# StefanSko/mcmc-db

Hardware: AMD Instinct MI355X
Metric: validated param-draws/sec (higher is better)
Workload: dtype f64; 1 GPU; single posteriordb-shaped model, 4x10000x100 synthetic draws per GPU (BASELINE config 1; AR(1) chains, ties and a shifted chain; SURVEY 8(d) C1); layout=pcn, statistics=mean,std,q5,q50,q95,split_rhat,ess_bulk,ess_tail

## Files before the change

### mcmc-db_amd/csrc/mcr_device.hpp

```cpp
#pragma once
#include <hip/hip_runtime.h>
#include <stdint.h>

namespace mcr {

using i64 = long long;
using u32 = unsigned int;
using u64 = unsigned long long;

constexpr int kWave = 64;

template <int CTRL>
__device__ __forceinline__ double dpp_f64(double v)
{
    const int lo = __builtin_amdgcn_mov_dpp(__double2loint(v), CTRL, 0xf, 0xf, true);
    const int hi = __builtin_amdgcn_mov_dpp(__double2hiint(v), CTRL, 0xf, 0xf, true);
    return __hiloint2double(hi, lo);
}
__device__ __forceinline__ double readlane_f64(double v, int lane)
{
    return __hiloint2double(__builtin_amdgcn_readlane(__double2hiint(v), lane),
                            __builtin_amdgcn_readlane(__double2loint(v), lane));
}
constexpr int kDppXor1 = 0xB1, kDppXor2 = 0x4E, kDppRor4 = 0x124, kDppRor8 = 0x128;

__device__ __forceinline__ double row_sum(double v)
{
    v += dpp_f64<kDppXor1>(v); v += dpp_f64<kDppXor2>(v); v += dpp_f64<kDppRor4>(v); v += dpp_f64<kDppRor8>(v);
    return v;
}
template <int CTRL>
__device__ __forceinline__ u32 dpp_u32(u32 v) { return (u32)__builtin_amdgcn_mov_dpp((int)v, CTRL, 0xf, 0xf, true); }
__device__ __forceinline__ u32 row_min_u32(u32 v)
{
    v = min(v, dpp_u32<kDppXor1>(v)); v = min(v, dpp_u32<kDppXor2>(v));
    v = min(v, dpp_u32<kDppRor4>(v)); v = min(v, dpp_u32<kDppRor8>(v));
    return v;
}
__device__ __forceinline__ u32 row_max_u32(u32 v)
{
    v = max(v, dpp_u32<kDppXor1>(v)); v = max(v, dpp_u32<kDppXor2>(v));
    v = max(v, dpp_u32<kDppRor4>(v)); v = max(v, dpp_u32<kDppRor8>(v));
    return v;
}
__device__ __forceinline__ double wave_sum(double v)
{
    v = row_sum(v);
    return (readlane_f64(v, 0) + readlane_f64(v, 16)) + (readlane_f64(v, 32) + readlane_f64(v, 48));
}
template <int CTRL, int ROW_MASK>
__device__ __forceinline__ double dpp_f64_or_zero(double v)
{
    const int lo = __builtin_amdgcn_update_dpp(0, __double2loint(v), CTRL, ROW_MASK, 0xf, false);
    const int hi = __builtin_amdgcn_update_dpp(0, __double2hiint(v), CTRL, ROW_MASK, 0xf, false);
    return __hiloint2double(hi, lo);
}
__device__ __forceinline__ double wave_excl_scan(double v, double& total)
{
    double incl = v;
    incl += dpp_f64_or_zero<0x111, 0xf>(incl);
    incl += dpp_f64_or_zero<0x112, 0xf>(incl);
    incl += dpp_f64_or_zero<0x114, 0xf>(incl);
    incl += dpp_f64_or_zero<0x118, 0xf>(incl);
    incl += dpp_f64_or_zero<0x142, 0xa>(incl);
    incl += dpp_f64_or_zero<0x143, 0xc>(incl);
    total = readlane_f64(incl, 63);
    return incl - v;
}

__device__ __forceinline__ int row_lane(int v, int j)
{
#define MCR_RL(J) case J: return __builtin_amdgcn_update_dpp(0, v, 0x150 + J, 0xf, 0xf, false);
    switch (j & 15) {
        MCR_RL(0) MCR_RL(1) MCR_RL(2) MCR_RL(3) MCR_RL(4) MCR_RL(5) MCR_RL(6) MCR_RL(7)
        MCR_RL(8) MCR_RL(9) MCR_RL(10) MCR_RL(11) MCR_RL(12) MCR_RL(13) MCR_RL(14)
        default: return __builtin_amdgcn_update_dpp(0, v, 0x15F, 0xf, 0xf, false);
    }
#undef MCR_RL
}

template <int CTRL, int ROW_MASK, int OLD>
__device__ __forceinline__ int dpp_i32_or(int v) { return __builtin_amdgcn_update_dpp(OLD, v, CTRL, ROW_MASK, 0xf, false); }

__device__ __forceinline__ u32 wave_excl_scan_u32(u32 v, u32& total)
{
    int incl = (int)v;
    incl += dpp_i32_or<0x111, 0xf, 0>(incl); incl += dpp_i32_or<0x112, 0xf, 0>(incl);
    incl += dpp_i32_or<0x114, 0xf, 0>(incl); incl += dpp_i32_or<0x118, 0xf, 0>(incl);
    incl += dpp_i32_or<0x142, 0xa, 0>(incl);
    incl += dpp_i32_or<0x143, 0xc, 0>(incl);
    total = (u32)__builtin_amdgcn_readlane(incl, 63);
    return (u32)incl - v;
}

__device__ __forceinline__ int wave_prefix_max(int v, int& excl)
{
    v = max(v, dpp_i32_or<0x111, 0xf, -1>(v)); v = max(v, dpp_i32_or<0x112, 0xf, -1>(v));
    v = max(v, dpp_i32_or<0x114, 0xf, -1>(v)); v = max(v, dpp_i32_or<0x118, 0xf, -1>(v));
    v = max(v, dpp_i32_or<0x142, 0xa, -1>(v)); v = max(v, dpp_i32_or<0x143, 0xc, -1>(v));
    excl = dpp_i32_or<0x138, 0xf, -1>(v);
    return v;
}
__device__ __forceinline__ int wave_suffix_min(int v, int& excl)
{
    constexpr int kMax = 0x7fffffff;
    v = min(v, dpp_i32_or<0x101, 0xf, kMax>(v)); v = min(v, dpp_i32_or<0x102, 0xf, kMax>(v));
    v = min(v, dpp_i32_or<0x104, 0xf, kMax>(v)); v = min(v, dpp_i32_or<0x108, 0xf, kMax>(v));
    const int r1 = __builtin_amdgcn_readlane(v, 16), r2 = __builtin_amdgcn_readlane(v, 32), r3 = __builtin_amdgcn_readlane(v, 48);
    const int row = (threadIdx.x & 63) >> 4;
    const int m23 = min(r2, r3), m123 = min(r1, m23);
    const int above = (row == 0) ? m123 : ((row == 1) ? m23 : ((row == 2) ? r3 : kMax));
    v = min(v, above);
    excl = dpp_i32_or<0x130, 0xf, kMax>(v);
    return v;
}

template <int NT>
__device__ __forceinline__ double block_sum(double v, double* red)
{
    v = wave_sum(v);
    __syncthreads();
    if ((threadIdx.x & 63) == 0) red[threadIdx.x >> 6] = v;
    __syncthreads();
    double r = 0.0;
#pragma unroll
    for (int w = 0; w < NT / kWave; ++w) r += red[w];
    return r;
}

template <int NT>
__device__ __forceinline__ void block_sum3(double& a, double& b, double& c, double* red)
{
    constexpr int NW = NT / kWave;
    a = wave_sum(a); b = wave_sum(b); c = wave_sum(c);
    __syncthreads();
    if ((threadIdx.x & 63) == 0) {
        const int w = threadIdx.x >> 6;
        red[w] = a; red[NW + w] = b; red[2 * NW + w] = c;
    }
    __syncthreads();
    double ra = 0.0, rb = 0.0, rc = 0.0;
#pragma unroll
    for (int w = 0; w < NW; ++w) { ra += red[w]; rb += red[NW + w]; rc += red[2 * NW + w]; }
    a = ra; b = rb; c = rc;
    __syncthreads();
}

__device__ __noinline__ double inv_cdf(double p)
{
#pragma clang fp contract(off)
    double q = p - 0.5, r, num, den, x;
    if (fabs(q) <= 0.425) {
        r = 0.180625 - q * q;
        num = (((((((2.5090809287301226727e+3 * r + 3.3430575583588128105e+4) * r +
                    6.7265770927008700853e+4) * r + 4.5921953931549871457e+4) * r +
                  1.3731693765509461125e+4) * r + 1.9715909503065514427e+3) * r +
                1.3314166789178437745e+2) * r + 3.3871328727963666080e+0) * q;
        den = (((((((5.2264952788528545610e+3 * r + 2.8729085735721942674e+4) * r +
                    3.9307895800092710610e+4) * r + 2.1213794301586595867e+4) * r +
                  5.3941960214247511077e+3) * r + 6.8718700749205790830e+2) * r +
                4.2313330701600911252e+1) * r + 1.0);
        return num / den;
    }
    r = (q <= 0.0) ? p : 1.0 - p;
    r = sqrt(-log(r));
    if (r <= 5.0) {
        r = r - 1.6;
        num = (((((((7.74545014278341407640e-4 * r + 2.27238449892691845833e-2) * r +
                    2.41780725177450611770e-1) * r + 1.27045825245236838258e+0) * r +
                  3.64784832476320460504e+0) * r + 5.76949722146069140550e+0) * r +
                4.63033784615654529590e+0) * r + 1.42343711074968357734e+0);
        den = (((((((1.05075007164441684324e-9 * r + 5.47593808499534494600e-4) * r +
                    1.51986665636164571966e-2) * r + 1.48103976427480074590e-1) * r +
                  6.89767334985100004550e-1) * r + 1.67638483018380384940e+0) * r +
                2.05319162663775882187e+0) * r + 1.0);
    } else {
        r = r - 5.0;
        num = (((((((2.01033439929228813265e-7 * r + 2.71155556874348757815e-5) * r +
                    1.24266094738807843860e-3) * r + 2.65321895265761230930e-2) * r +
                  2.96560571828504891230e-1) * r + 1.78482653991729133580e+0) * r +
                5.46378491116411436990e+0) * r + 6.65790464350110377720e+0);
        den = (((((((2.04426310338993978564e-15 * r + 1.42151175831644588870e-7) * r +
                    1.84631831751005468180e-5) * r + 7.86869131145613259100e-4) * r +
                  1.48753612908506148525e-2) * r + 1.36929880922735805310e-1) * r +
                5.99832206555887937690e-1) * r + 1.0);
    }
    x = num / den;
    return (q < 0.0) ? -x : x;
}

template <class FA, class FB>
__device__ __forceinline__ i64 merge_path(FA a, i64 na, FB b, i64 nb, i64 diag)
{
    i64 lo = diag > nb ? diag - nb : 0;
    i64 hi = diag < na ? diag : na;
    while (lo < hi) {
        i64 mid = (lo + hi) >> 1;
        const auto ak = a(mid), bk = b(diag - 1 - mid);
        if (!(bk < ak)) lo = mid + 1; else hi = mid;
    }
    return lo;
}

template <class FA, class FB>
__device__ __forceinline__ int merge_path32(FA a, int na, FB b, int nb, int diag)
{
    int lo = diag > nb ? diag - nb : 0;
    int hi = diag < na ? diag : na;
    while (lo < hi) {
        const int mid = (lo + hi) >> 1;
        const auto ak = a(mid), bk = b(diag - 1 - mid);
        const bool right = !(bk < ak);
        lo = right ? mid + 1 : lo;
        hi = right ? hi : mid;
    }
    return lo;
}

template <class FA, class FB>
__device__ __forceinline__ i64 merge_path_wave(FA a, i64 na, FB b, i64 nb, i64 diag)
{
    const int lane = threadIdx.x & 63;
    i64 lo = diag > nb ? diag - nb : 0;
    i64 hi = diag < na ? diag : na;
    while (lo < hi) {
        const i64 span = hi - lo;
        const bool small = span <= 64;
        const i64 mid = small ? lo + lane : lo + (span * (lane + 1)) / 65;
        bool pred = false;
        if (!small || lane < span) pred = !(b(diag - 1 - mid) < a(mid));
        const int cnt = __popcll(__ballot(pred));
        if (small) { lo += cnt; hi = lo; }
        else {
            const i64 nlo = (cnt == 0) ? lo : lo + (span * (i64)cnt) / 65 + 1;
            const i64 nhi = (cnt == 64) ? hi : lo + (span * (i64)(cnt + 1)) / 65;
            lo = nlo; hi = nhi;
        }
    }
    return lo;
}

__device__ __forceinline__ int pos16(int e) { return e ^ ((e >> 4) & 15); }
__device__ __forceinline__ int posi(int e) { return e ^ ((e >> 5) & 15); }

__device__ __forceinline__ u32 f32_key(float x)
{
    u32 b = __float_as_uint(x);
    if (x == 0.0f) b = 0u;
    return (b & 0x80000000u) ? ~b : (b | 0x80000000u);
}
__device__ __forceinline__ double key_value(u32 k)
{
    const u32 b = (k & 0x80000000u) ? (k ^ 0x80000000u) : ~k;
    return (double)__uint_as_float(b);
}
constexpr u64 kRecPad = ~0ull;

__device__ __forceinline__ double sorted_key(const double* a, i64 i) { return a[i]; }
__device__ __forceinline__ double sorted_key(const u64* a, i64 i) { return key_value((u32)(a[i] >> 32)); }

__host__ __device__ __forceinline__ u64 splitmix64(u64 x)
{
    u64 z = x + 0x9E3779B97F4A7C15ull;
    z = (z ^ (z >> 30)) * 0xBF58476D1CE4E5B9ull;
    z = (z ^ (z >> 27)) * 0x94D049BB133111EBull;
    return z ^ (z >> 31);
}

}
```

### mcmc-db_amd/csrc/mcr_kernels.hpp

```cpp
#pragma once
#include "mcr_device.hpp"
#include "mcr_sortnet.h"

namespace mcr {

enum ResField {
    R_MEAN = 0, R_STD, R_MEDIAN, R_RHAT, R_RHAT_BULK, R_RHAT_TAIL, R_ESS_BULK, R_ESS_TAIL,
    R_LAG_BULK, R_LAG_TAIL, R_BAD, R_Q0
};

#ifndef MCR_WCOMB
#define MCR_WCOMB 1
#endif
constexpr bool kWriteCombine = MCR_WCOMB != 0;

struct QArgs {
    int nq;
    i64 lo[32];
    double g[32];
};

__device__ __forceinline__ bool xcd_map(i64 P, int nb, i64& p, int& blk)
{
    const i64 L = blockIdx.x;
// ... 130 lines not shown
#pragma unroll
            for (int j = 0; j < V; ++j) acc1((double)v[j]);
        }
        scalar_from = b + nvec * V;
    }
    for (i64 j = scalar_from + threadIdx.x; j < e; j += 256) acc1((double)x[j]);
    block_sum3<256>(s1, s2, bad, red);
    if (threadIdx.x == 0) store_slice_moments(part + (p * S + s) * kMomRec, K, s1, s2, bad, (double)(e > b ? e - b : 0));
}

template <typename T>
__global__ __launch_bounds__(256) void k_moments_cols(const T* __restrict__ src, i64 C, i64 N, i64 P,
                                                      i64 sc, i64 sn, i64 sp, double* __restrict__ part,
                                                      int S)
{
    __shared__ double sh[3][4][64];
    const int tx = threadIdx.x & 63, ty = threadIdx.x >> 6;
    const i64 p = (i64)blockIdx.x * 64 + tx;
    const int s = blockIdx.y;
    const i64 M = C * N;
    const i64 per = (M + S - 1) / S, b = s * per, e = (b + per < M) ? b + per : M;
    double s1 = 0.0, s2 = 0.0, bad = 0.0, K = 0.0;
    if (p < P && b < e) {
        { const i64 c = b / N, t = b - c * N; K = (double)src[c * sc + t * sn + p * sp]; }
        if (!isfinite(K)) K = 0.0;
        for (i64 r = b + ty; r < e; r += 4) {
            const i64 c = r / N, t = r - c * N;
            const double v = (double)src[c * sc + t * sn + p * sp], d = v - K;
            s1 += d; s2 = fma(d, d, s2);
            bad += isfinite(v) ? 0.0 : 1.0;
        }
    }
    sh[0][ty][tx] = s1; sh[1][ty][tx] = s2; sh[2][ty][tx] = bad;
    __syncthreads();
    if (ty == 0 && p < P)
        store_slice_moments(part + (p * S + s) * kMomRec, K, sh[0][0][tx] + sh[0][1][tx] + sh[0][2][tx] + sh[0][3][tx],
                            sh[1][0][tx] + sh[1][1][tx] + sh[1][2][tx] + sh[1][3][tx],
                            sh[2][0][tx] + sh[2][1][tx] + sh[2][2][tx] + sh[2][3][tx], (double)(e > b ? e - b : 0));
}

__global__ void k_moments_final(const double* __restrict__ part, int S, i64 P, double* __restrict__ mean,
                                double* __restrict__ stdv, double* __restrict__ bad)
{
    const i64 p = (i64)blockIdx.x * blockDim.x + threadIdx.x;
    if (p >= P) return;
    double mu, m2, b, n;
    merge_slice_moments(part + p * S * kMomRec, S, mu, m2, b, n);
    double var = m2 / n;
    if (isinf(m2)) var = INFINITY;
    else if (!(var >= 0.0)) var = 0.0;
    mean[p] = mu;
    stdv[p] = sqrt(var);
    if (bad) bad[p] = b;
}

template <int VT>
__device__ __forceinline__ void thread_sort(double (&k)[VT], u32 (&ix)[VT])
{
    static_assert(VT == 16 || VT == 8, "sorting networks exist for 16 and 8 items per lane");
#define MCR_CE(a, b)                                                        \
    {                                                                       \
        const bool sw = k[b] < k[a];                                        \
        const double lo = sw ? k[b] : k[a], hi = sw ? k[a] : k[b];          \
        const u32 ilo = sw ? ix[b] : ix[a], ihi = sw ? ix[a] : ix[b];       \
        k[a] = lo; k[b] = hi; ix[a] = ilo; ix[b] = ihi;                     \
    }
    if constexpr (VT == 16) { MCR_NET16(MCR_CE) } else { MCR_NET8(MCR_CE) }
#undef MCR_CE
}

#ifndef MCR_TILE_DPP_LEVELS
#define MCR_TILE_DPP_LEVELS 3
#endif

__device__ __forceinline__ u32 select_by_mask(u32 a, u32 b, unsigned long long m)
{
    u32 r;
    asm("v_cndmask_b32_e64 %0, %1, %2, %3" : "=v"(r) : "v"(a), "v"(b), "s"(m));
    return r;
}
__device__ __forceinline__ double select_by_mask(double a, double b, unsigned long long m)
{
    return __hiloint2double((int)select_by_mask((u32)__double2hiint(a), (u32)__double2hiint(b), m),
                            (int)select_by_mask((u32)__double2loint(a), (u32)__double2loint(b), m));
}

template <int CTRL, bool MIRROR, unsigned long long MIN_LANES>
__device__ __forceinline__ void lane_pair_stage(double (&k)[16], u32 (&ix)[16])
{
    auto exchange = [](double& own, u32& own_i, double o, u32 oi) {
        const unsigned long long lt = __builtin_amdgcn_ballot_w64(o < own), gt = __builtin_amdgcn_ballot_w64(own < o);
        const unsigned long long take = (lt & MIN_LANES) | (gt & ~MIN_LANES);
        own = select_by_mask(own, o, take);
        own_i = select_by_mask(own_i, oi, take);
    };
#pragma unroll
    for (int r = 0; r < (MIRROR ? 8 : 16); ++r) {
        const int s = MIRROR ? 15 - r : r;
        const double o_r = dpp_f64<CTRL>(k[s]);
        const u32 oi_r = dpp_u32<CTRL>(ix[s]);
        if (MIRROR) {
            const double o_s = dpp_f64<CTRL>(k[r]);
            const u32 oi_s = dpp_u32<CTRL>(ix[r]);
            exchange(k[s], ix[s], o_s, oi_s);
        }
        exchange(k[r], ix[r], o_r, oi_r);
    }
}

__device__ __forceinline__ void lane_bitonic_merge16(double (&k)[16], u32 (&ix)[16])
{
#define MCR_CE(a, b)                                                        \
    {                                                                       \
        const bool sw = k[b] < k[a];                                        \
        const double lo = sw ? k[b] : k[a], hi = sw ? k[a] : k[b];          \
        const u32 ilo = sw ? ix[b] : ix[a], ihi = sw ? ix[a] : ix[b];       \
        k[a] = lo; k[b] = hi; ix[a] = ilo; ix[b] = ihi;                     \
    }
    MCR_BITONIC16(MCR_CE)
#undef MCR_CE
}

__device__ __forceinline__ void lane_merge_levels_16_to_64(double (&k)[16], u32 (&ix)[16])
{
    constexpr unsigned long long kEvenLanes = 0x5555555555555555ull, kLowPairs = 0x3333333333333333ull;
    lane_pair_stage<0xB1, true, kEvenLanes>(k, ix);
    lane_bitonic_merge16(k, ix);
    lane_pair_stage<0x1B, true, kLowPairs>(k, ix);
    lane_pair_stage<0xB1, false, kEvenLanes>(k, ix);
    lane_bitonic_merge16(k, ix);
#if MCR_TILE_DPP_LEVELS >= 3
    constexpr unsigned long long kLowQuads = 0x0F0F0F0F0F0F0F0Full;
    lane_pair_stage<0x141, true, kLowQuads>(k, ix);
    lane_pair_stage<0x4E, false, kLowPairs>(k, ix);
    lane_pair_stage<0xB1, false, kEvenLanes>(k, ix);
    lane_bitonic_merge16(k, ix);
#endif
}

template <int VT>
__device__ __forceinline__ void serial_merge(const double* skey, int a0, int na, int b0, int nb, int ai,
                                             int bi, int nout, double (&k)[VT], int (&src)[VT])
{
    int pa = a0 + ai, pb = b0 + bi;
    const int ea = a0 + na, eb = b0 + nb;
    double ak = skey[pos16(pa)], bk = skey[pos16(pb)];
#pragma unroll
    for (int i = 0; i < VT; ++i) {
        if (i < nout) {
            const bool takeA = (pb >= eb) | ((pa < ea) & !(bk < ak));
            k[i] = takeA ? ak : bk;
            src[i] = takeA ? pa : pb;
            pa += takeA ? 1 : 0;
            pb += takeA ? 0 : 1;
            const int pn = takeA ? pa : pb;
            const double nv = skey[pos16(pn)];
            ak = takeA ? nv : ak;
            bk = takeA ? bk : nv;
        } else {
            src[i] = 0;
        }
    }
}

template <typename IdxT> constexpr size_t sort_lds_bytes(int T) { return (size_t)T * (8 + sizeof(IdxT)); }

template <int NT, int VT, typename IdxT, typename XT>
__global__ __launch_bounds__(NT) void k_tile_sort(const XT* __restrict__ X, i64 M,
                                                  double* __restrict__ keys, IdxT* __restrict__ idx,
                                                  double* __restrict__ part, int ntiles,
                                                  double* __restrict__ samp)
{
    constexpr int T = NT * VT;
    extern __shared__ __attribute__((aligned(16))) char smem[];
    double* skey = reinterpret_cast<double*>(smem);
    IdxT* sidx = reinterpret_cast<IdxT*>(skey + T);
    double* red = skey;

    const int tid = threadIdx.x, tile = blockIdx.x;
    const i64 p = blockIdx.y;
    const i64 base = (i64)tile * T;
    const int count = (int)((M - base < (i64)T) ? M - base : (i64)T);
    const XT* src = X + p * M + base;

    double bad = 0.0;
#pragma unroll
    for (int i = 0; i < VT; ++i) {
        const int e = i * NT + tid;
        double v = INFINITY;
        if (e < count) {
            v = (double)src[e];
            bad += isfinite(v) ? 0.0 : 1.0;
        }
        skey[pos16(e)] = v;
    }
    __syncthreads();

    double k[VT];
    u32 ix[VT];
#pragma unroll
    for (int i = 0; i < VT; ++i) {
        const int e = tid * VT + i;
        k[i] = skey[pos16(e)];
        ix[i] = (e < count) ? (u32)(base + e) : 0xFFFFFFFFu;
    }
    thread_sort<VT>(k, ix);
    constexpr bool kLaneLevels = MCR_TILE_DPP_LEVELS >= 2 && VT == 16;
    if constexpr (kLaneLevels) lane_merge_levels_16_to_64(k, ix);
    __syncthreads();
#pragma unroll
    for (int i = 0; i < VT; ++i) {
        const int e = tid * VT + i;
        skey[pos16(e)] = k[i];
        sidx[posi(e)] = (IdxT)ix[i];
    }
    __syncthreads();

    for (int coop = kLaneLevels ? (MCR_TILE_DPP_LEVELS >= 3 ? 16 : 8) : 2; coop <= NT; coop <<= 1) {
        const int first = tid & ~(coop - 1);
        const int run = VT * (coop >> 1);
        const int a0 = first * VT, b0 = a0 + run;
        const int diag = VT * (tid - first);
        auto A = [&](int i) { return skey[pos16(a0 + i)]; };
        auto B = [&](int j) { return skey[pos16(b0 + j)]; };
        const int ai = merge_path32(A, run, B, run, diag);
        int srcs[VT];
        serial_merge<VT>(skey, a0, run, b0, run, ai, diag - ai, VT, k, srcs);
#pragma unroll
        for (int i = 0; i < VT; ++i) ix[i] = sidx[posi(srcs[i])];
        __syncthreads();
#pragma unroll
        for (int i = 0; i < VT; ++i) {
            const int e = tid * VT + i;
            skey[pos16(e)] = k[i];
            sidx[posi(e)] = (IdxT)ix[i];
        }
        __syncthreads();
    }

    for (int e = tid; e < count; e += NT) {
        keys[p * M + base + e] = skey[pos16(e)];
        idx[p * M + base + e] = sidx[posi(e)];
    }
    if (samp != nullptr && tid < T / 64) {
        const int e = 64 * tid + 63;
        samp[(p * ntiles + tile) * (T / 64) + tid] = (e < count) ? skey[pos16(e)] : INFINITY;
    }
    __syncthreads();
    double s1 = 0.0;
#pragma unroll
    for (int i = 0; i < VT; ++i) s1 += (tid * VT + i < count) ? k[i] : 0.0;
    s1 = block_sum<NT>(s1, red);
    const double mt = s1 / (double)count;
    double s2 = 0.0, e1 = 0.0;
#pragma unroll
    for (int i = 0; i < VT; ++i) { const double d = (tid * VT + i < count) ? k[i] - mt : 0.0; s2 = fma(d, d, s2); e1 += d; }
    block_sum3<NT>(s2, e1, bad, red);
    if (tid == 0) store_slice_moments(part + (p * ntiles + tile) * kMomRec, mt, e1, s2, bad, (double)count);
}

template <int NT, int VT>
__device__ __forceinline__ void scatter_codes_by_line(u32* __restrict__ zrow, i64 M, int total, const u32 (&hcode)[VT],
                                                      const u32 (&hpos)[VT], u32* cnt_code, unsigned short* spos, u32* swt)
{
    constexpr int kMaxLines = 2048, PER = kMaxLines / NT > 0 ? kMaxLines / NT : 1;
    static_assert(NT * PER >= kMaxLines, "every line counter has an owner in the scan");
    const int tid = threadIdx.x;
    const int nlines = (int)((M + 31) >> 5);
    u32* scnt = cnt_code;
    u32* scode = cnt_code + 2112;
    __syncthreads();
    for (int i = tid; i <= nlines; i += NT) scnt[i] = 0u;
    __syncthreads();
    u32 rk[VT];
#pragma unroll
    for (int i = 0; i < VT; ++i) rk[i] = (tid * VT + i < total) ? atomicAdd(&scnt[hpos[i] >> 5], 1u) : 0u;
    __syncthreads();
    {
        u32 c[PER], tsum = 0;
#pragma unroll
        for (int j = 0; j < PER; ++j) { const int q = tid * PER + j; c[j] = (q < nlines) ? scnt[q] : 0u; tsum += c[j]; }
        u32 wtot;
        const u32 wex = wave_excl_scan_u32(tsum, wtot);
        if ((tid & 63) == 0) swt[tid >> 6] = wtot;
        __syncthreads();
        u32 base = wex;
        for (int w = 0; w < (tid >> 6); ++w) base += swt[w];
#pragma unroll
        for (int j = 0; j < PER; ++j) { const int q = tid * PER + j; if (q < nlines) scnt[q] = base; base += c[j]; }
    }
    __syncthreads();
#pragma unroll
    for (int i = 0; i < VT; ++i) {
        if (tid * VT + i < total) {
            const u32 slot = min(scnt[hpos[i] >> 5] + rk[i], (u32)(NT * VT - 1));
            scode[slot] = hcode[i];
            spos[slot] = (unsigned short)hpos[i];
        }
    }
    __syncthreads();
    for (int e = tid; e < total; e += NT) zrow[spos[e]] = scode[e];
}

template <int NT, int VT, class KF>
__device__ __forceinline__ void block_tie_runs(KF key_at, int total, int* wsh, int (&rs)[VT], int (&re)[VT])
{
    constexpr int NW = NT / kWave;
    const int tid = threadIdx.x, lane = tid & 63, w = tid >> 6;
    const int base = tid * VT;
    bool h[VT];
    auto prev = key_at((base > 0 && base - 1 < total) ? base - 1 : 0);
    int cur = -1, first = 0x7fffffff;
#pragma unroll
    for (int i = 0; i < VT; ++i) {
        const int g = base + i;
        const auto kv = key_at(g < total ? g : 0);
        h[i] = (g == 0) || (g >= total) || (prev != kv);
        if (h[i]) { cur = g; if (first == 0x7fffffff) first = g; }
        rs[i] = cur;
        prev = kv;
    }
    int exL, exR;
    const int incl = wave_prefix_max(cur, exL);
    const int rinc = wave_suffix_min(first, exR);
    __syncthreads();
    if (lane == 63) wsh[w] = incl;
    if (lane == 0) wsh[NW + w] = rinc;
    __syncthreads();
    int carryL = -1, carryR = total;
#pragma unroll
    for (int ww = 0; ww < NW; ++ww) {
        if (ww < w) carryL = max(carryL, wsh[ww]);
        if (ww > w) carryR = min(carryR, wsh[NW + ww]);
    }
    carryL = max(carryL, exL);
    carryR = min(carryR, exR);
    if (carryR > total) carryR = total;
    int nxt = carryR;
#pragma unroll
    for (int i = VT - 1; i >= 0; --i) {
        re[i] = nxt;
        if (h[i]) nxt = base + i;
        if (rs[i] < 0) rs[i] = carryL;
    }
    __syncthreads();
}

template <typename KT>
__device__ __forceinline__ i64 wave_order_stats(const KT* __restrict__ k, i64 M, const QArgs& q, bool write,
                                                double* __restrict__ res, i64 P, i64 p, double& med_out)
{
#pragma clang fp contract(off)
    const int lane = threadIdx.x & 63;
    if (write && lane < q.nq) {
        const int j = lane;
        const i64 lo = q.lo[j], hi = (lo + 1 < M) ? lo + 1 : M - 1;
        const double a = sorted_key(k, lo), b = sorted_key(k, hi), d = b - a, g = q.g[j];
        res[(R_Q0 + j) * P + p] = (g >= 0.5) ? b - d * (1.0 - g) : a + d * g;
    }
    const double below = (M >= 2) ? sorted_key(k, M / 2 - 1) : -INFINITY, at = sorted_key(k, M / 2);
    const double med = (M & 1) ? at : (below + at) / 2.0;
    if (write && lane == 0) res[R_MEDIAN * P + p] = med;
    if (below < med && !(at < med)) { med_out = med; return M / 2; }
    i64 lo = 0, hi = M;
    while (lo < hi) {
        const i64 step = (hi - lo + 63) / 64;
        const i64 pos = lo + step * (lane + 1) - 1;
        const bool less = (pos < hi) && (sorted_key(k, pos) < med);
        const i64 cnt = (i64)__popcll(__ballot(less));
        const i64 nhi = lo + step * (cnt + 1) - 1;
        lo += step * cnt;
        hi = (nhi < hi) ? nhi : hi;
    }
    med_out = med;
    return lo;
}

template <int NT, int VT, bool FOLD, typename IdxT, typename KT = double>
__global__ __launch_bounds__(NT) void k_merge(const KT* __restrict__ kin, const IdxT* __restrict__ iin,
                                              double* __restrict__ kout, IdxT* __restrict__ iout, i64 M,
                                              i64 R, double* __restrict__ res, i64 P,
                                              QArgs q, u32* __restrict__ z, const i64* __restrict__ split_in)
{
    constexpr int OBS = NT * VT;
    constexpr int OB = FOLD ? OBS - 64 : OBS;
    extern __shared__ __attribute__((aligned(16))) char smem[];
    double* skey = reinterpret_cast<double*>(smem);
    IdxT* sidx = reinterpret_cast<IdxT*>(skey + OBS);
    i64* sh = FOLD ? reinterpret_cast<i64*>(skey + OB) : reinterpret_cast<i64*>(sidx + OBS);

    const int tid = threadIdx.x;
    i64 p = blockIdx.y;
    int blk = blockIdx.x;
    if (FOLD) {
        if (!xcd_map(P, (int)((M + OB - 1) / OB), p, blk)) return;
    }
    const i64 o0 = (i64)blk * OB;
    if (o0 >= M) return;
    const KT* kp = kin + p * M;
    const IdxT* ip = iin + p * M;
    auto KEY = [&](i64 g) -> double { return sorted_key(kp, g); };
    auto POS = [&](i64 g) -> u32 {
        if constexpr (sizeof(KT) == 8 && !__is_same(KT, double)) return (u32)kp[g]; else return (u32)ip[g];
    };

    i64 abase, na, bbase, nb, d0;
    double med = 0.0;
    if (!FOLD) {
        const i64 pb = (o0 / (2 * R)) * (2 * R);
        abase = pb;
        na = (M - pb < R) ? M - pb : R;
        bbase = pb + na;
        nb = (M - bbase < R) ? M - bbase : R;
        d0 = o0 - pb;
    } else {
        if (split_in != nullptr) {
            if (tid == 0) { sh[0] = split_in[p]; reinterpret_cast<double*>(sh)[1] = res[R_MEDIAN * P + p]; }
        } else if (tid < 64) {
            double m_;
            const i64 s_ = wave_order_stats(kp, M, q, blk == 0, res, P, p, m_);
            if (tid == 0) { sh[0] = s_; reinterpret_cast<double*>(sh)[1] = m_; }
        }
        __syncthreads();
        const i64 s = sh[0];
        med = reinterpret_cast<double*>(sh)[1];
        __syncthreads();
        abase = s - 1;
        na = s;
        bbase = s;
        nb = M - s;
        d0 = o0;
    }
    const i64 tot = na + nb;
    const i64 d1 = (d0 + OB < tot) ? d0 + OB : tot;

    auto GA = [&](i64 i) -> double { return FOLD ? med - KEY(abase - i) : KEY(abase + i); };
    auto GB = [&](i64 j) -> double { return FOLD ? KEY(bbase + j) - med : KEY(bbase + j); };
    if (tid < 64) { const i64 r0 = merge_path_wave(GA, na, GB, nb, d0); if (tid == 0) sh[0] = r0; }
    else if (tid < 128) { const i64 r1 = merge_path_wave(GA, na, GB, nb, d1); if (tid == 64) sh[1] = r1; }
    __syncthreads();
    const i64 ai0 = sh[0], ai1 = sh[1];
    const i64 bi0 = d0 - ai0;
    const int ca = (int)(ai1 - ai0), cb = (int)((d1 - ai1) - bi0);
    const int total = ca + cb;

    {
        double gv[VT]; u32 gi[VT];
#pragma unroll
        for (int j = 0; j < VT; ++j) {
            const int e = j * NT + tid;
            const bool inA = e < ca;
            i64 g = inA ? (FOLD ? abase - (ai0 + e) : abase + ai0 + e) : bbase + bi0 + (e - ca);
            g = (e < total) ? g : 0;
            const double x = KEY(g);
            gv[j] = FOLD ? (inA ? med - x : x - med) : x;
            gi[j] = POS(g);
        }
#pragma unroll
        for (int j = 0; j < VT; ++j) {
            const int e = j * NT + tid;
            if (e < total) { skey[pos16(e)] = gv[j]; sidx[posi(e)] = (IdxT)gi[j]; }
        }
    }
    __syncthreads();

    const int diag = (tid * VT < total) ? tid * VT : total;
    const int nout = (total - diag < VT) ? total - diag : VT;
    auto A = [&](int i) { return skey[pos16(i)]; };
    auto B = [&](int j) { return skey[pos16(ca + j)]; };
    const int ai = merge_path32(A, ca, B, cb, diag);
    double k[VT];
    int srcs[VT];
    u32 ix[VT];
    serial_merge<VT>(skey, 0, ca, ca, cb, ai, diag - ai, nout, k, srcs);
#pragma unroll
    for (int i = 0; i < VT; ++i) ix[i] = sidx[posi(srcs[i])];
    __syncthreads();
#pragma unroll
    for (int i = 0; i < VT; ++i) {
        if (i < nout) {
            skey[pos16(diag + i)] = k[i];
            sidx[posi(diag + i)] = (IdxT)ix[i];
        }
    }
    __syncthreads();
    if (z == nullptr) {
        for (int e = tid; e < total; e += NT) {
            kout[p * M + o0 + e] = skey[pos16(e)];
            iout[p * M + o0 + e] = sidx[posi(e)];
        }
        return;
    }
    if (tid == 0) {
        const i64 bi1 = d1 - ai1;
        const double v0 = skey[pos16(0)], v1 = skey[pos16(total - 1)];
        bool ext0 = false, ext1 = false;
        if (ai0 > 0 && GA(ai0 - 1) == v0) ext0 = true;
        if (bi0 > 0 && GB(bi0 - 1) == v0) ext0 = true;
        if (ai1 < na && GA(ai1) == v1) ext1 = true;
        if (bi1 < nb && GB(bi1) == v1) ext1 = true;
        sh[2] = ext0; sh[3] = ext1;
    }
    __syncthreads();
    const bool ext0 = sh[2] != 0, ext1 = sh[3] != 0;
    __syncthreads();
    if ((ext0 || ext1) && tid < 8) {
        const int which = tid >> 2, side = (tid >> 1) & 1, upper = tid & 1;
        const double v = which ? skey[pos16(total - 1)] : skey[pos16(0)];
        const i64 len = side ? nb : na;
        i64 lo = 0, hi = len;
        while (lo < hi) {
            const i64 mid = (lo + hi) >> 1;
            const double x = side ? GB(mid) : GA(mid);
            const bool right = upper ? !(v < x) : (x < v);
            if (right) lo = mid + 1; else hi = mid;
        }
        sh[2 + tid] = lo;
    }
    __syncthreads();
    const double vfirst = skey[pos16(0)], vlast = skey[pos16(total - 1)];
    const i64 gfirst = sh[2 + 0] + sh[2 + 2];
    const i64 glast = sh[2 + 5] + sh[2 + 7];
    int rs[VT], re[VT];
    block_tie_runs<NT, VT>([&](int g) { return skey[pos16(g)]; }, total, reinterpret_cast<int*>(sh + 12), rs, re);
    const bool by_line = kWriteCombine && M <= 65535;
    u32 hcode[VT], hpos[VT];
#pragma unroll
    for (int i = 0; i < VT; ++i) {
        const int e = tid * VT + i;
        hcode[i] = 0u; hpos[i] = 0u;
        if (e < total) {
            const double v = skey[pos16(e)];
            i64 gs = d0 + rs[i], ge = d0 + re[i];
            if (ext0 && v == vfirst) gs = gfirst;
            if (ext1 && v == vlast) ge = glast;
            const u32 t_idx = min((u32)sidx[posi(e)], (u32)(M - 1));
            hcode[i] = (u32)(gs + ge); hpos[i] = t_idx;
            if (!by_line) z[p * M + t_idx] = (u32)(gs + ge);
        }
    }
    if (by_line)
        scatter_codes_by_line<NT, VT>(z + p * M, M, total, hcode, hpos, reinterpret_cast<u32*>(skey),
                                      reinterpret_cast<unsigned short*>(sidx), reinterpret_cast<u32*>(sh));
}

constexpr int kMaxBucketTiles = 16;

__host__ __device__ inline size_t splitters_base_bytes(int S, int B, int k, int mvt)
{
    const size_t base = (size_t)S * (mvt > 0 ? 8 : 12) + (size_t)(B + 1) * 16 + (size_t)(B + 1) * k * 4 + 64;
    return (base + 15) / 16 * 16;
}
__host__ __device__ inline size_t splitters_lds_bytes(int S, int B, int k, int mvt)
{
    return splitters_base_bytes(S, B, k, mvt) + (mvt > 0 ? (size_t)(1024 * mvt + 16) * 10 : 0);
}

template <typename KT, int MVT>
__global__ __launch_bounds__(1024) void k_splitters(const KT* __restrict__ keys,
                                                    const double* __restrict__ samp, i64 M, int k, int B,
                                                    int D, i64 R, u32* __restrict__ cut, u32* __restrict__ boff)
{
    constexpr int NTS = 1024;
    const int SPT = (int)(R / 64);
    const int S = k * SPT;
    extern __shared__ __attribute__((aligned(16))) char smem[];
    double* sv = reinterpret_cast<double*>(smem);
    double* splv = sv + S;
    int* srank = reinterpret_cast<int*>(splv + B + 1);
    int* splt = srank + (MVT > 0 ? 0 : S);
    int* splp = splt + B + 1;
    u32* scut = reinterpret_cast<u32*>(splp + B + 1);
    const int tid = threadIdx.x;
    const i64 p = blockIdx.x;
    const KT* kp = keys + p * M;
    for (int i = tid; i < S; i += NTS) { sv[i] = samp[p * S + i]; if (MVT == 0) srank[i] = i % SPT; }
    for (int b = tid; b <= B; b += NTS) splt[b] = -1;
    if (MVT > 0) {
        constexpr int VT = MVT > 0 ? MVT : 1;
        static_assert(MVT == 0 || 64 % VT == 0, "a thread's VT outputs must not straddle two pairs of runs (run lengths are multiples of 64)");
        constexpr int SP = NTS * VT;
        double* mk = reinterpret_cast<double*>(smem + splitters_base_bytes(S, B, k, MVT));
        unsigned short* mi = reinterpret_cast<unsigned short*>(mk + SP + 16);
        for (int e = tid; e < SP + 16; e += NTS) {
            mk[pos16(e)] = (e < S) ? samp[p * S + e] : INFINITY;
            mi[e] = (unsigned short)(e < S ? e : 0xFFFF);
        }
        __syncthreads();
        const int chunk0 = tid * VT;
        for (int g = SPT; g < SP; g <<= 1) {
            double kk[VT]; int srcs[VT]; unsigned short ids[VT];
            const int a0 = chunk0 / (2 * g) * (2 * g);
            const int a1 = (a0 + g < SP) ? a0 + g : SP, b1 = (a0 + 2 * g < SP) ? a0 + 2 * g : SP;
            const int na = a1 - a0, nb = b1 - a1, diag = chunk0 - a0;
            const bool moved = nb > 0;
            if (moved) {
                auto A = [&](int i) { return mk[pos16(a0 + i)]; };
                auto Bf = [&](int j) { return mk[pos16(a1 + j)]; };
                const int ai = merge_path32(A, na, Bf, nb, diag);
                serial_merge<VT>(mk, a0, na, a1, nb, ai, diag - ai, VT, kk, srcs);
#pragma unroll
                for (int i = 0; i < VT; ++i) ids[i] = mi[srcs[i]];
            }
            __syncthreads();
            if (moved) {
#pragma unroll
                for (int i = 0; i < VT; ++i) { mk[pos16(chunk0 + i)] = kk[i]; mi[chunk0 + i] = ids[i]; }
            }
            __syncthreads();
        }
        for (int b = 1 + tid; b < B; b += NTS) {
            const int r = b * D - 1;
            if (r < SP) {
                const double v = mk[pos16(r)];
                const int i = mi[r];
                if (v < INFINITY && i < S) { splv[b] = v; splt[b] = i / SPT; splp[b] = 64 * (i % SPT) + 63; }
            }
        }
        __syncthreads();
    } else {
    __syncthreads();
    for (i64 q = tid; q < (i64)S * k; q += NTS) {
        const int t2 = (int)(q / S), i = (int)(q - (i64)t2 * S);
        const double v = sv[i];
        const int t = i / SPT;
        if (t2 == t || !(v < INFINITY)) continue;
        const double* a = sv + t2 * SPT;
        int lo = 0, hi = SPT;
        if (t2 < t) { while (lo < hi) { const int m = (lo + hi) >> 1; if (!(v < a[m])) lo = m + 1; else hi = m; } }
        else        { while (lo < hi) { const int m = (lo + hi) >> 1; if (a[m] < v) lo = m + 1; else hi = m; } }
        if (lo) atomicAdd(&srank[i], lo);
    }
    __syncthreads();
    for (int i = tid; i < S; i += NTS) {
        if (!(sv[i] < INFINITY)) continue;
        const int r = srank[i];
        if ((r + 1) % D == 0) {
            const int b = (r + 1) / D;
            if (b >= 1 && b < B) { splv[b] = sv[i]; splt[b] = i / SPT; splp[b] = 64 * (i % SPT) + 63; }
        }
    }
    __syncthreads();
    }
    {
        int missing = 0;
        for (int b = 1 + tid; b < B; b += NTS) missing |= (splt[b] < 0);
        if (__syncthreads_or(missing)) {
            for (int q = tid; q < (B + 1) * k; q += NTS) cut[p * (i64)(B + 1) * k + q] = 0u;
            for (int b = tid; b <= B; b += NTS) boff[p * (B + 1) + b] = 0u;
            return;
        }
    }
    for (int q = tid; q < (B + 1) * k; q += NTS) {
        const int b = q / k, t = q % k;
        const i64 tbase = (i64)t * R;
        const int cnt = (int)((M - tbase < R) ? M - tbase : R);
        u32 c;
        if (b == 0) c = 0;
        else if (b == B) c = (u32)cnt;
        else {
            const double v = splv[b];
            const int ts = splt[b];
            if (t == ts) c = (u32)(splp[b] + 1);
            else {
                const double* sa = sv + t * SPT;
                int slo = 0, shi = SPT;
                if (t < ts) { while (slo < shi) { const int m = (slo + shi) >> 1; if (!(v < sa[m])) slo = m + 1; else shi = m; } }
                else        { while (slo < shi) { const int m = (slo + shi) >> 1; if (sa[m] < v) slo = m + 1; else shi = m; } }
                const KT* a = kp + tbase;
                int lo = 64 * slo, hi = 64 * slo + 63;
                if (lo > cnt) lo = cnt;
                if (hi > cnt) hi = cnt;
                if (t < ts) { while (lo < hi) { const int m = (lo + hi) >> 1; if (!(v < sorted_key(a, m))) lo = m + 1; else hi = m; } }
                else        { while (lo < hi) { const int m = (lo + hi) >> 1; if (sorted_key(a, m) < v) lo = m + 1; else hi = m; } }
                c = (u32)lo;
            }
        }
        scut[q] = c;
        cut[(p * (B + 1) + b) * k + t] = c;
    }
    __syncthreads();
    for (int b = tid; b <= B; b += NTS) {
        u32 o = 0;
        for (int t = 0; t < k; ++t) o += scut[b * k + t];
        boff[p * (B + 1) + b] = o;
    }
}

template <typename KT>
__global__ __launch_bounds__(256) void k_sample_runs(const KT* __restrict__ keys, i64 M, i64 R,
                                                     double* __restrict__ samp)
{
    const int run = blockIdx.x, k = gridDim.x;
    const i64 p = blockIdx.y;
    const int SPT = (int)(R / 64);
    const i64 base = (i64)run * R;
    for (int j = threadIdx.x; j < SPT; j += 256) {
        const i64 e = base + 64 * (i64)j + 63;
        samp[(p * k + run) * SPT + j] = (e < M && 64 * (i64)j + 63 < R) ? sorted_key(keys, p * M + e) : INFINITY;
    }
}

template <int NT, int VT, typename IdxT>
__global__ __launch_bounds__(NT) void k_bucket_merge(const double* __restrict__ kin, const IdxT* __restrict__ iin,
                                                      double* __restrict__ kout, IdxT* __restrict__ iout, i64 M,
                                                      int k, int B, const u32* __restrict__ cut,
                                                      const u32* __restrict__ boff, u32* __restrict__ z, i64 P,
                                                      i64 R)
{
    constexpr int T = NT * VT;
    static_assert(T == 4096, "the partition bound of k_splitters assumes 4096-slot buckets");
    extern __shared__ __attribute__((aligned(16))) char smem[];
    double* skey = reinterpret_cast<double*>(smem);
    IdxT* sidx = reinterpret_cast<IdxT*>(skey + T);
    int* sst = reinterpret_cast<int*>(skey + (T - 64));
    int* spl = sst + 40;
    int* sps = spl + 40;
    i64* sedge = reinterpret_cast<i64*>(sps + 40);

    const int tid = threadIdx.x;
    i64 p;
    int b;
    if (!xcd_map(P, B, p, b)) return;
    const double* kp = kin + p * M;
    const IdxT* ip = iin + p * M;
    const u32* c0 = cut + (p * (B + 1) + b) * k;
    const u32* c1 = c0 + k;
    if (tid == 0) {
        int acc = 0;
        for (int t = 0; t < k; ++t) {
            const int len = (int)(c1[t] - c0[t]);
            sst[t] = acc; spl[t] = len; sps[t] = (int)c0[t];
            acc += (len + 15) & ~15;
        }
        sst[k] = acc;
    }
    __syncthreads();
    const int padded = sst[k];
    const int total = (int)(boff[p * (B + 1) + b + 1] - boff[p * (B + 1) + b]);
    const i64 obase = boff[p * (B + 1) + b];
    if (padded > T - 64 || total < 0 || total > padded || obase + total > M) return;
    {
        const int lane = tid & 63, wv = tid >> 6;
        u32 my_g = 0; int my_n = 0;
        if ((lane & 15) < VT) {
            const int e0 = (lane & 15) * NT + 64 * wv + 16 * (lane >> 4);
            if (e0 < padded) {
                int t = 0;
#pragma unroll
                for (int step = 8; step > 0; step >>= 1)
                    if (t + step < k && e0 >= sst[t + step]) t += step;
                const int o = e0 - sst[t];
                my_n = spl[t] - o;
                my_g = (u32)((i64)t * R) + (u32)sps[t] + (u32)o;
            }
        }
        double gv[VT]; IdxT gi[VT];
#pragma unroll
        for (int j = 0; j < VT; ++j) {
            const int within = lane & 15;
            const u32 g0 = (u32)row_lane((int)my_g, j);
            const int n = row_lane(my_n, j);
            const bool live = within < n;
            const i64 g = live ? (i64)(g0 + (u32)within) : 0;
            const double v = kp[g]; const IdxT id = ip[g];
            gv[j] = live ? v : INFINITY; gi[j] = live ? id : (IdxT)~(IdxT)0;
        }
#pragma unroll
        for (int j = 0; j < VT; ++j) {
            const int e = j * NT + tid;
            if (e < padded) { skey[pos16(e)] = gv[j]; sidx[posi(e)] = gi[j]; }
        }
    }
    __syncthreads();
    const int chunk0 = tid * VT;
    int mypiece = 0;
#pragma unroll
    for (int step = 8; step > 0; step >>= 1)
        if (mypiece + step < k && chunk0 >= sst[mypiece + step]) mypiece += step;
    for (int w = 1; w < k; w <<= 1) {
        double kk[VT]; int srcs[VT]; u32 ix[VT];
        const bool active = chunk0 < padded;
        bool moved = false;
        if (active) {
            const int ra = mypiece & ~(2 * w - 1);
            const int a0 = sst[ra];
            const int a1 = sst[(ra + w < k) ? ra + w : k];
            const int b1 = sst[(ra + 2 * w < k) ? ra + 2 * w : k];
            const int na = a1 - a0, nb = b1 - a1, diag = chunk0 - a0;
            moved = nb > 0;
            if (moved) {
                auto A = [&](int i) { return skey[pos16(a0 + i)]; };
                auto Bf = [&](int j) { return skey[pos16(a1 + j)]; };
                const int ai = merge_path32(A, na, Bf, nb, diag);
                serial_merge<VT>(skey, a0, na, a1, nb, ai, diag - ai, VT, kk, srcs);
#pragma unroll
                for (int i = 0; i < VT; ++i) ix[i] = sidx[posi(srcs[i])];
            }
        }
        __syncthreads();
        if (moved) {
#pragma unroll
            for (int i = 0; i < VT; ++i) { skey[pos16(chunk0 + i)] = kk[i]; sidx[posi(chunk0 + i)] = (IdxT)ix[i]; }
        }
        __syncthreads();
    }
    for (int e = tid; e < total; e += NT) {
        kout[p * M + obase + e] = skey[pos16(e)];
        iout[p * M + obase + e] = sidx[posi(e)];
    }
    if (z == nullptr || total == 0) return;
    if (tid < 4) sedge[tid] = 0;
    if (tid < 64) {
        bool e0 = false, e1 = false;
        if (tid < k) {
            const i64 tbase = (i64)tid * R;
            const int cnt = (int)((M - tbase < R) ? M - tbase : R);
            const int lo = sps[tid], hi = sps[tid] + spl[tid];
            if (lo > 0) e0 = (kp[tbase + lo - 1] == skey[pos16(0)]);
            if (hi < cnt) e1 = (kp[tbase + hi] == skey[pos16(total - 1)]);
        }
        const bool a0 = __ballot(e0) != 0, a1 = __ballot(e1) != 0;
        if (tid == 0) { sst[36] = a0; sst[37] = a1; }
    }
    __syncthreads();
    const bool ext0 = sst[36] != 0, ext1 = sst[37] != 0;
    if ((ext0 || ext1) && tid < 2 * k) {
        const int t = tid % k, which = tid / k;
        const double v = which ? skey[pos16(total - 1)] : skey[pos16(0)];
        const i64 tbase = (i64)t * R;
        const int cnt = (int)((M - tbase < R) ? M - tbase : R);
        const double* a = kp + tbase;
        int lo = 0, hi = cnt;
        while (lo < hi) { const int m = (lo + hi) >> 1; if (a[m] < v) lo = m + 1; else hi = m; }
        const int lb = lo;
        hi = cnt;
        while (lo < hi) { const int m = (lo + hi) >> 1; if (!(v < a[m])) lo = m + 1; else hi = m; }
        atomicAdd(reinterpret_cast<unsigned long long*>(&sedge[2 * which]), (unsigned long long)lb);
        atomicAdd(reinterpret_cast<unsigned long long*>(&sedge[2 * which + 1]), (unsigned long long)lo);
    }
    __syncthreads();
    const double vfirst = skey[pos16(0)], vlast = skey[pos16(total - 1)];
    int rs[VT], re[VT];
    block_tie_runs<NT, VT>([&](int g) { return skey[pos16(g)]; }, total, sst + 24, rs, re);
#pragma unroll
    for (int i = 0; i < VT; ++i) {
        const int e = tid * VT + i;
        if (e < total) {
            const double v = skey[pos16(e)];
            i64 gs = obase + rs[i], ge = obase + re[i];
            if (ext0 && v == vfirst) gs = sedge[0];
            if (ext1 && v == vlast) ge = sedge[3];
            z[p * M + min((u32)sidx[posi(e)], (u32)(M - 1))] = (u32)(gs + ge);
        }
    }
}

template <typename KT>
__global__ __launch_bounds__(256) void k_order_stats(const KT* __restrict__ keys, i64 M, i64 P, QArgs q,
                                                     double* __restrict__ res, i64* __restrict__ split)
{
    const int lane = threadIdx.x & 63;
    const i64 p = (i64)blockIdx.x * 4 + (threadIdx.x >> 6);
    if (p >= P) return;
    double med;
    const i64 s = wave_order_stats(keys + p * M, M, q, true, res, P, p, med);
    if (lane == 0) split[p] = s;
}

__global__ __launch_bounds__(256) void k_rank_z(const double* __restrict__ keys,
                                                const u32* __restrict__ idx, i64 M, u32* __restrict__ z)
{
    const i64 p = blockIdx.y;
    const i64 i = (i64)blockIdx.x * 256 + threadIdx.x;
    if (i >= M) return;
    const double* k = keys + p * M;
    const double v = k[i];
    i64 s = i, e = i + 1;
    if (i > 0 && k[i - 1] == v) {
        i64 step = 1, hi = i - 1;
        i64 lo = hi - step;
        while (lo >= 0 && k[lo] == v) { hi = lo; step <<= 1; lo = hi - step; }
        if (lo < -1) lo = -1;
        while (hi - lo > 1) {
            const i64 mid = (lo + hi) >> 1;
            if (k[mid] == v) hi = mid; else lo = mid;
        }
        s = hi;
    }
    if (i + 1 < M && k[i + 1] == v) {
        i64 step = 1, lo = i + 1;
        i64 hi = lo + step;
        while (hi < M && k[hi] == v) { lo = hi; step <<= 1; hi = lo + step; }
        if (hi > M) hi = M;
        while (hi - lo > 1) {
            const i64 mid = (lo + hi) >> 1;
            if (k[mid] == v) lo = mid; else hi = mid;
        }
        e = lo + 1;
    }
    z[p * M + min(idx[p * M + i], (u32)(M - 1))] = (u32)(s + e);
}

__device__ __forceinline__ void finalize_param(const double* __restrict__ part, int S, i64 M,
                                               i64 P, int C, double* __restrict__ res, i64 p)
{
    double mu, m2, b, n;
    merge_slice_moments(part + p * S * kMomRec, S, mu, m2, b, n);
    double var = m2 / (double)M;
    if (isinf(m2)) var = INFINITY;
    else if (!(var >= 0.0)) var = 0.0;
    res[R_MEAN * P + p] = mu;
    res[R_STD * P + p] = sqrt(var);
    res[R_BAD * P + p] = b;
    if (C < 2) {
        res[R_RHAT * P + p] = NAN; res[R_RHAT_BULK * P + p] = NAN; res[R_RHAT_TAIL * P + p] = NAN;
        res[R_ESS_BULK * P + p] = NAN; res[R_ESS_TAIL * P + p] = NAN;
        res[R_LAG_BULK * P + p] = 0.0; res[R_LAG_TAIL * P + p] = 0.0;
    } else {
        const double rb = res[R_RHAT_BULK * P + p], rt = res[R_RHAT_TAIL * P + p];
        res[R_RHAT * P + p] = (rt > rb) ? rt : rb;
    }
}

__global__ void k_finalize(const double* __restrict__ part, int S, i64 M, i64 P, int C, double* __restrict__ res)
{
    const i64 p = (i64)blockIdx.x * blockDim.x + threadIdx.x;
    if (p >= P) return;
    finalize_param(part, S, M, P, C, res, p);
}

__global__ void k_compare(const double* __restrict__ ref, const double* __restrict__ act, i64 n,
                          double tol, double* __restrict__ rel, unsigned char* __restrict__ pass)
{
    const i64 i = (i64)blockIdx.x * blockDim.x + threadIdx.x;
    if (i >= n) return;
    const double r = ref[i], a = act[i], ar = fabs(r);
    const double denom = (1e-12 > ar) ? 1e-12 : ar;
    const double e = fabs(a - r) / denom;
    rel[i] = e;
    pass[i] = (e <= tol) ? 1 : 0;
}

__global__ __launch_bounds__(256) void k_stream_read(const uint4* __restrict__ src, i64 nvec, u32* __restrict__ sink)
{
    const i64 per = (nvec + gridDim.x - 1) / gridDim.x;
    const i64 b = (i64)blockIdx.x * per, e = (b + per < nvec) ? b + per : nvec;
    u32 acc = 0;
    i64 i = b + threadIdx.x;
    for (; i + 3 * 256 < e; i += 4 * 256) {
        uint4 r[4];
#pragma unroll
        for (int u = 0; u < 4; ++u) r[u] = src[i + u * 256];
#pragma unroll
        for (int u = 0; u < 4; ++u) acc ^= r[u].x ^ r[u].y ^ r[u].z ^ r[u].w;
    }
    for (; i < e; i += 256) { const uint4 r = src[i]; acc ^= r.x ^ r.y ^ r.z ^ r.w; }
    if (acc == 0x9E3779B9u) sink[blockIdx.x & 1023] = acc;
}

template <typename T>
__global__ __launch_bounds__(256) void k_fill_synth(T* __restrict__ out, i64 total, i64 M, u64 seed, i64 first)
{
    const i64 stride = (i64)gridDim.x * 256;
    for (i64 j = (i64)blockIdx.x * 256 + threadIdx.x; j < total; j += stride) {
        const i64 i = first + j;
        const i64 p = i / M;
        const u64 base = seed * 0x9E3779B97F4A7C15ull + 2ull * (u64)i;
        const u64 h1 = splitmix64(base), h2 = splitmix64(base + 1);
        const double u1 = ((double)(h1 >> 11) + 0.5) * 0x1.0p-53;
        const double u2 = (double)(h2 >> 11) * 0x1.0p-53;
        const double e = sqrt(-2.0 * log(u1)) * cospi(2.0 * u2);
        int k = (int)(p % 7) - 3;
        double sigma = 1.0;
        for (; k > 0; --k) sigma *= 10.0;
        for (; k < 0; ++k) sigma /= 10.0;
        out[j] = (T)((double)p + sigma * e);
    }
}

}
```

Baseline: 24.18 billion param-draws/s.

## Keep merged keys in registers for tie-run ranking, use bitmask run bounds

The fold path now computes tie runs straight from the per-thread merged registers instead of writing them back to LDS and reading them again. Run heads are stored as a bitmask and run starts and ends come from clz/ffs, which removes the per-element rs/re arrays. Neighbour keys are fetched with a DPP cross-lane move, and values read from shared memory are forced into scalar registers with readfirstlane. This cuts LDS round-trips, barriers and VGPR pressure, but depends on the register state being correct at the edges (the lane-0 previous key, padded elements, and the "moved" flag in the multi-piece merge).

```diff
diff --git a/mcmc-db_amd/csrc/mcr_device.hpp b/mcmc-db_amd/csrc/mcr_device.hpp
--- a/mcmc-db_amd/csrc/mcr_device.hpp
+++ b/mcmc-db_amd/csrc/mcr_device.hpp
@@ -21,6 +21,15 @@
 {
     return __hiloint2double(__builtin_amdgcn_readlane(__double2hiint(v), lane),
                             __builtin_amdgcn_readlane(__double2loint(v), lane));
+}
+__device__ __forceinline__ i64 uniform_i64(i64 v)
+{
+    return (i64)(((u64)(u32)__builtin_amdgcn_readfirstlane((int)((u64)v >> 32)) << 32) |
+                 (u64)(u32)__builtin_amdgcn_readfirstlane((int)(u64)v));
+}
+__device__ __forceinline__ double uniform_f64(double v)
+{
+    return __hiloint2double(__builtin_amdgcn_readfirstlane(__double2hiint(v)), __builtin_amdgcn_readfirstlane(__double2loint(v)));
 }
 constexpr int kDppXor1 = 0xB1, kDppXor2 = 0x4E, kDppRor4 = 0x124, kDppRor8 = 0x128;
 
diff --git a/mcmc-db_amd/csrc/mcr_kernels.hpp b/mcmc-db_amd/csrc/mcr_kernels.hpp
--- a/mcmc-db_amd/csrc/mcr_kernels.hpp
+++ b/mcmc-db_amd/csrc/mcr_kernels.hpp
@@ -456,28 +456,50 @@
     for (int e = tid; e < total; e += NT) zrow[spos[e]] = scode[e];
 }
 
-template <int NT, int VT, class KF>
-__device__ __forceinline__ void block_tie_runs(KF key_at, int total, int* wsh, int (&rs)[VT], int (&re)[VT])
+struct TieRuns {
+    u32 heads;
+    int base;
+    int carryL;
+    int carryR;
+    __device__ __forceinline__ int start(int i) const
+    {
+        const u32 m = heads & ((2u << i) - 1u);
+        return m ? base + 31 - __clz((int)m) : carryL;
+    }
+    __device__ __forceinline__ int end(int i) const
+    {
+        const u32 m = heads >> (i + 1);
+        return m ? base + i + __ffs((int)m) : carryR;
+    }
+};
+
+template <int VT, typename K, class KF>
+__device__ __forceinline__ u32 tie_heads(KF key_at, K prev, int total)
+{
+    static_assert(VT <= 32, "one bit per position");
+    const int base = threadIdx.x * VT;
+    u32 h = 0u;
+#pragma unroll
+    for (int i = 0; i < VT; ++i) {
+        const int g = base + i;
+        const K kv = key_at(i, g);
+        if ((g == 0) || (g >= total) || (prev != kv)) h |= 1u << i;
+        prev = kv;
+    }
+    return h;
+}
+
+template <int NT, int VT>
+__device__ __forceinline__ TieRuns tie_run_bounds(u32 heads, int total, int* wsh)
 {
     constexpr int NW = NT / kWave;
     const int tid = threadIdx.x, lane = tid & 63, w = tid >> 6;
     const int base = tid * VT;
-    bool h[VT];
-    auto prev = key_at((base > 0 && base - 1 < total) ? base - 1 : 0);
-    int cur = -1, first = 0x7fffffff;
-#pragma unroll
-    for (int i = 0; i < VT; ++i) {
-        const int g = base + i;
-        const auto kv = key_at(g < total ? g : 0);
-        h[i] = (g == 0) || (g >= total) || (prev != kv);
-        if (h[i]) { cur = g; if (first == 0x7fffffff) first = g; }
-        rs[i] = cur;
-        prev = kv;
-    }
+    const int cur = heads ? base + 31 - __clz((int)heads) : -1;
+    const int first = heads ? base + __ffs((int)heads) - 1 : 0x7fffffff;
     int exL, exR;
     const int incl = wave_prefix_max(cur, exL);
     const int rinc = wave_suffix_min(first, exR);
-    __syncthreads();
     if (lane == 63) wsh[w] = incl;
     if (lane == 0) wsh[NW + w] = rinc;
     __syncthreads();
@@ -490,14 +512,28 @@
     carryL = max(carryL, exL);
     carryR = min(carryR, exR);
     if (carryR > total) carryR = total;
-    int nxt = carryR;
-#pragma unroll
-    for (int i = VT - 1; i >= 0; --i) {
-        re[i] = nxt;
-        if (h[i]) nxt = base + i;
-        if (rs[i] < 0) rs[i] = carryL;
-    }
-    __syncthreads();
+    return TieRuns{heads, base, carryL, carryR};
+}
+
+template <int NT, int VT, class KF>
+__device__ __forceinline__ void block_tie_runs(KF key_at, int total, int* wsh, int (&rs)[VT], int (&re)[VT])
+{
+    const int base = threadIdx.x * VT;
+    const u32 heads = tie_heads<VT>([&](int, int g) { return key_at(g < total ? g : 0); },
+                                    key_at((base > 0 && base - 1 < total) ? base - 1 : 0), total);
+    __syncthreads();
+    const TieRuns tr = tie_run_bounds<NT, VT>(heads, total, wsh);
+    __syncthreads();
+#pragma unroll
+    for (int i = 0; i < VT; ++i) { rs[i] = tr.start(i); re[i] = tr.end(i); }
+}
+
+template <int NT, int VT>
+__device__ __forceinline__ TieRuns block_tie_runs_reg(const double (&k)[VT], double lane0_prev, int total, int* wsh)
+{
+    const double below = dpp_f64<0x138>(k[VT - 1]);
+    const u32 heads = tie_heads<VT>([&](int i, int) { return k[i]; }, (threadIdx.x & 63) ? below : lane0_prev, total);
+    return tie_run_bounds<NT, VT>(heads, total, wsh);
 }
 
 template <typename KT>
@@ -576,8 +612,8 @@
             if (tid == 0) { sh[0] = s_; reinterpret_cast<double*>(sh)[1] = m_; }
         }
         __syncthreads();
-        const i64 s = sh[0];
-        med = reinterpret_cast<double*>(sh)[1];
+        const i64 s = uniform_i64(sh[0]);
+        med = uniform_f64(reinterpret_cast<double*>(sh)[1]);
         __syncthreads();
         abase = s - 1;
         na = s;
@@ -593,7 +629,7 @@
     if (tid < 64) { const i64 r0 = merge_path_wave(GA, na, GB, nb, d0); if (tid == 0) sh[0] = r0; }
     else if (tid < 128) { const i64 r1 = merge_path_wave(GA, na, GB, nb, d1); if (tid == 64) sh[1] = r1; }
     __syncthreads();
-    const i64 ai0 = sh[0], ai1 = sh[1];
+    const i64 ai0 = uniform_i64(sh[0]), ai1 = uniform_i64(sh[1]);
     const i64 bi0 = d0 - ai0;
     const int ca = (int)(ai1 - ai0), cb = (int)((d1 - ai1) - bi0);
     const int total = ca + cb;
@@ -629,25 +665,44 @@
     serial_merge<VT>(skey, 0, ca, ca, cb, ai, diag - ai, nout, k, srcs);
 #pragma unroll
     for (int i = 0; i < VT; ++i) ix[i] = sidx[posi(srcs[i])];
-    __syncthreads();
-#pragma unroll
-    for (int i = 0; i < VT; ++i) {
-        if (i < nout) {
-            skey[pos16(diag + i)] = k[i];
-            sidx[posi(diag + i)] = (IdxT)ix[i];
-        }
-    }
-    __syncthreads();
-    if (z == nullptr) {
+    if (!FOLD) {
+        __syncthreads();
+#pragma unroll
+        for (int i = 0; i < VT; ++i) {
+            if (i < nout) {
+                skey[pos16(diag + i)] = k[i];
+                sidx[posi(diag + i)] = (IdxT)ix[i];
+            }
+        }
+        __syncthreads();
         for (int e = tid; e < total; e += NT) {
             kout[p * M + o0 + e] = skey[pos16(e)];
             iout[p * M + o0 + e] = sidx[posi(e)];
         }
         return;
     }
+    double* const wlast = reinterpret_cast<double*>(sh + 20);
+    double* const vedge = reinterpret_cast<double*>(sh + 20 + NT / kWave);
+    static_assert(20 + NT / kWave + 2 <= 64, "the fold's scratch fits the 64 freed key slots");
+    if ((tid & 63) == 63) wlast[tid >> 6] = k[VT - 1];
+    if (tid == 0) vedge[0] = k[0];
+    if (nout > 0 && diag + nout == total) {
+        double v = k[0];
+#pragma unroll
+        for (int i = 1; i < VT; ++i) v = (i == nout - 1) ? k[i] : v;
+        vedge[1] = v;
+    }
+    __syncthreads();
+    const double vfirst = vedge[0], vlast = vedge[1];
+    u32 at_edge = 0u;
+#pragma unroll
+    for (int i = 0; i < VT; ++i) at_edge |= ((k[i] == vfirst) ? 1u << i : 0u) | ((k[i] == vlast) ? 1u << (VT + i) : 0u);
+    asm volatile("" : "+v"(at_edge));
+    const double lane0_prev = ((tid & 63) == 0 && tid > 0) ? wlast[(tid >> 6) - 1] : 0.0;
+    const TieRuns tr = block_tie_runs_reg<NT, VT>(k, lane0_prev, total, reinterpret_cast<int*>(sh + 12));
     if (tid == 0) {
         const i64 bi1 = d1 - ai1;
-        const double v0 = skey[pos16(0)], v1 = skey[pos16(total - 1)];
+        const double v0 = vedge[0], v1 = vedge[1];
         bool ext0 = false, ext1 = false;
         if (ai0 > 0 && GA(ai0 - 1) == v0) ext0 = true;
         if (bi0 > 0 && GB(bi0 - 1) == v0) ext0 = true;
@@ -660,7 +715,7 @@
     __syncthreads();
     if ((ext0 || ext1) && tid < 8) {
         const int which = tid >> 2, side = (tid >> 1) & 1, upper = tid & 1;
-        const double v = which ? skey[pos16(total - 1)] : skey[pos16(0)];
+        const double v = vedge[which];
         const i64 len = side ? nb : na;
         i64 lo = 0, hi = len;
         while (lo < hi) {
@@ -672,11 +727,8 @@
         sh[2 + tid] = lo;
     }
     __syncthreads();
-    const double vfirst = skey[pos16(0)], vlast = skey[pos16(total - 1)];
     const i64 gfirst = sh[2 + 0] + sh[2 + 2];
     const i64 glast = sh[2 + 5] + sh[2 + 7];
-    int rs[VT], re[VT];
-    block_tie_runs<NT, VT>([&](int g) { return skey[pos16(g)]; }, total, reinterpret_cast<int*>(sh + 12), rs, re);
     const bool by_line = kWriteCombine && M <= 65535;
     u32 hcode[VT], hpos[VT];
 #pragma unroll
@@ -684,11 +736,10 @@
         const int e = tid * VT + i;
         hcode[i] = 0u; hpos[i] = 0u;
         if (e < total) {
-            const double v = skey[pos16(e)];
-            i64 gs = d0 + rs[i], ge = d0 + re[i];
-            if (ext0 && v == vfirst) gs = gfirst;
-            if (ext1 && v == vlast) ge = glast;
-            const u32 t_idx = min((u32)sidx[posi(e)], (u32)(M - 1));
+            i64 gs = d0 + tr.start(i), ge = d0 + tr.end(i);
+            if (ext0 && (at_edge >> i & 1u)) gs = gfirst;
+            if (ext1 && (at_edge >> (VT + i) & 1u)) ge = glast;
+            const u32 t_idx = min(ix[i], (u32)(M - 1));
             hcode[i] = (u32)(gs + ge); hpos[i] = t_idx;
             if (!by_line) z[p * M + t_idx] = (u32)(gs + ge);
         }
@@ -932,10 +983,12 @@
 #pragma unroll
     for (int step = 8; step > 0; step >>= 1)
         if (mypiece + step < k && chunk0 >= sst[mypiece + step]) mypiece += step;
+    double kk[VT]; u32 ix[VT];
+    bool moved = false;
     for (int w = 1; w < k; w <<= 1) {
-        double kk[VT]; int srcs[VT]; u32 ix[VT];
+        int srcs[VT];
         const bool active = chunk0 < padded;
-        bool moved = false;
+        moved = false;
         if (active) {
             const int ra = mypiece & ~(2 * w - 1);
             const int a0 = sst[ra];
@@ -995,17 +1048,21 @@
     }
     __syncthreads();
     const double vfirst = skey[pos16(0)], vlast = skey[pos16(total - 1)];
-    int rs[VT], re[VT];
-    block_tie_runs<NT, VT>([&](int g) { return skey[pos16(g)]; }, total, sst + 24, rs, re);
+    if (!moved && chunk0 < total) {
+#pragma unroll
+        for (int i = 0; i < VT; ++i) { kk[i] = skey[pos16(chunk0 + i)]; ix[i] = (u32)sidx[posi(chunk0 + i)]; }
+    }
+    const double lane0_prev = ((tid & 63) == 0 && tid > 0) ? skey[pos16(chunk0 - 1)] : 0.0;
+    const TieRuns tr = block_tie_runs_reg<NT, VT>(kk, lane0_prev, total, sst + 24);
 #pragma unroll
     for (int i = 0; i < VT; ++i) {
         const int e = tid * VT + i;
         if (e < total) {
-            const double v = skey[pos16(e)];
-            i64 gs = obase + rs[i], ge = obase + re[i];
+            const double v = kk[i];
+            i64 gs = obase + tr.start(i), ge = obase + tr.end(i);
             if (ext0 && v == vfirst) gs = sedge[0];
             if (ext1 && v == vlast) ge = sedge[3];
-            z[p * M + min((u32)sidx[posi(e)], (u32)(M - 1))] = (u32)(gs + ge);
+            z[p * M + min(ix[i], (u32)(M - 1))] = (u32)(gs + ge);
         }
     }
 }
```

New measurement: 24.56 billion param-draws/s, median of 6. 1.6% higher.
